# GradientSpaces/LivingScenes

Measured on AMD Instinct MI355X. Metric: object-instances/sec (encode+match+register), N=1024 pts, higher is better.
Workload: dtype f32 (GEMM products as two-piece f16 splits on the f16 matrix cores, fp32 accumulate: as accurate against fp64 as an fp32 FMA chain)

## Files before the change

livingscenes_amd/csrc/edge_fused.hip:

```cpp
#include "ls_common.h"

namespace ls {

constexpr int FK = 16;
constexpr int FND = 32;
typedef _Float16 fh8_t __attribute__((ext_vector_type(8)));
typedef _Float16 fh2_t __attribute__((ext_vector_type(2)));
typedef float ff2_t __attribute__((ext_vector_type(2)));
typedef float ff16_t __attribute__((ext_vector_type(16)));

__device__ __forceinline__ void fsplit_pair(ff2_t v, unsigned& h, unsigned& l) {
    const fh2_t hv = __builtin_convertvector(v, fh2_t);
    const fh2_t lv = __builtin_convertvector(v - __builtin_convertvector(hv, ff2_t), fh2_t);
    h = __builtin_bit_cast(unsigned, hv);
    l = __builtin_bit_cast(unsigned, lv);
}
__device__ __forceinline__ void fpow2(float amax, float& s, int& e_inv) {
    unsigned be = (__float_as_uint(amax) >> 23) & 0xffu;
    be = be < 15u ? 15u : be;
    s = __uint_as_float((268u - be) << 23);
    e_inv = (int)be - 14 - 127;
}
template <int CTRL>
__device__ __forceinline__ float fdpp_max(float v) {
    return fmaxf(v, __int_as_float(__builtin_amdgcn_update_dpp(__float_as_int(v), __float_as_int(v), CTRL, 0xF, 0xF, false)));
}
template <int CTRL>
__device__ __forceinline__ float fdpp_add(float v) {
    return v + __int_as_float(__builtin_amdgcn_update_dpp(0, __float_as_int(v), CTRL, 0xF, 0xF, true));
}
__device__ __forceinline__ float fquad_sum(float v) { return fdpp_add<0x4E>(fdpp_add<0xB1>(v)); }
__device__ __forceinline__ float fquad_max(float v) { return fdpp_max<0x4E>(fdpp_max<0xB1>(v)); }
__device__ __forceinline__ float finv_fro(float ss) { return __builtin_amdgcn_rsqf(fmaxf(ss, 1e-24f)); }

__global__ __launch_bounds__(64) void edge_ft_presplit_w_kernel(const float* __restrict__ W, int Co, int Cin, int KS, uint4* __restrict__ planes,
                                                                int* __restrict__ wexp) {
    const int T = blockIdx.x / KS, ks = blockIdx.x % KS, lane = threadIdx.x;
    const int head = T / 5, p = T % 5, r = lane & 31;
    const float* wr = W + ((size_t)(2 * p + (r >> 4)) * Co + 16 * head + (r & 15)) * Cin;
    float am = 0.f;
    for (int c = 0; c < Cin; ++c) am = fmaxf(am, fabsf(wr[c]));
    float sc;
    int e;
    fpow2(am, sc, e);
    if (ks == 0 && lane < 32) wexp[T * 32 + r] = e;
    const int k = ks * 16 + 8 * (lane >> 5);
    uint4 h, l;
    fsplit_pair(ff2_t{wr[k] * sc, wr[k + 1] * sc}, h.x, l.x);
    fsplit_pair(ff2_t{wr[k + 2] * sc, wr[k + 3] * sc}, h.y, l.y);
    fsplit_pair(ff2_t{wr[k + 4] * sc, wr[k + 5] * sc}, h.z, l.z);
    fsplit_pair(ff2_t{wr[k + 6] * sc, wr[k + 7] * sc}, h.w, l.w);
    planes[((size_t)blockIdx.x * 2) * 64 + lane] = h;
    planes[((size_t)blockIdx.x * 2 + 1) * 64 + lane] = l;
}
size_t edge_ft_w_bytes(int Co, int Cin) { return (size_t)(Co / 16) * 5 * (Cin / 16) * 2 * 64 * sizeof(uint4) + (size_t)(Co / 16) * 5 * 32 * sizeof(int); }
int edge_ft_presplit_w_launch(const float* W, int Co, int Cin, void* planes, hipStream_t st) {
    const int tiles = (Co / 16) * 5, KS = Cin / 16;
    hipLaunchKernelGGL(edge_ft_presplit_w_kernel, dim3(tiles * KS), dim3(64), 0, st, W, Co, Cin, KS, (uint4*)planes,
                       (int*)((uint4*)planes + (size_t)tiles * KS * 128));
    LS_LAUNCH_CHECK();
    return LS_OK;
}

template <int KS>
__global__ __launch_bounds__(256) void edge_ft_prep_a_kernel(const float* __restrict__ cur, const int32_t* __restrict__ rows, int Ns, int Nd,
                                                             uint4* __restrict__ planes, int* __restrict__ aexp) {
    constexpr int CIN = KS * 16, KPW = KS / 4;
    __shared__ float lmax[4][32];
    const int lane = threadIdx.x & 63, w = threadIdx.x >> 6, j = lane & 31, h = lane >> 5;
    const int R = blockIdx.x * 32 + j;
    size_t src = (size_t)R;
    if (rows) {
        const int x = R % 3, pn = R / 3, b = pn / Nd;
        src = ((size_t)b * Ns + rows[pn]) * 3 + x;
    }
    const float* rp = cur + src * CIN + (w * KPW) * 16 + h * 8;
    float4 v[KPW][2];
    float am = 0.f;
#pragma unroll
    for (int kk = 0; kk < KPW; ++kk) {
        v[kk][0] = *reinterpret_cast<const float4*>(rp + kk * 16);
        v[kk][1] = *reinterpret_cast<const float4*>(rp + kk * 16 + 4);
    }
#pragma unroll
    for (int kk = 0; kk < KPW; ++kk)
#pragma unroll
        for (int u = 0; u < 2; ++u)
            am = fmaxf(am, fmaxf(fmaxf(fabsf(v[kk][u].x), fabsf(v[kk][u].y)), fmaxf(fabsf(v[kk][u].z), fabsf(v[kk][u].w))));
    am = fmaxf(am, __shfl_xor(am, 32, 64));
    if (h == 0) lmax[w][j] = am;
    __syncthreads();
    am = fmaxf(fmaxf(lmax[0][j], lmax[1][j]), fmaxf(lmax[2][j], lmax[3][j]));
    float sc;
    int e;
    fpow2(am, sc, e);
    if (w == 0 && h == 0) aexp[R] = e;
#pragma unroll
    for (int kk = 0; kk < KPW; ++kk) {
        uint4 hh, ll;
        fsplit_pair(ff2_t{v[kk][0].x * sc, v[kk][0].y * sc}, hh.x, ll.x);
        fsplit_pair(ff2_t{v[kk][0].z * sc, v[kk][0].w * sc}, hh.y, ll.y);
        fsplit_pair(ff2_t{v[kk][1].x * sc, v[kk][1].y * sc}, hh.z, ll.z);
        fsplit_pair(ff2_t{v[kk][1].z * sc, v[kk][1].w * sc}, hh.w, ll.w);
        uint4* op = planes + (((size_t)blockIdx.x * KS + w * KPW + kk) * 2) * 64 + lane;
        op[0] = hh;
        op[64] = ll;
    }
}

struct FT43 { float4 x, y, z; };
__device__ __forceinline__ FT43 ft_lds43(const float* p, int sld) {
    FT43 r;
    r.x = *reinterpret_cast<const float4*>(p);
    r.y = *reinterpret_cast<const float4*>(p + sld);
    r.z = *reinterpret_cast<const float4*>(p + 2 * sld);
    return r;
}
__device__ __forceinline__ FT43 ft_add43(const FT43& a, const FT43& b) {
    FT43 r;
    r.x = make_float4(a.x.x + b.x.x, a.x.y + b.x.y, a.x.z + b.x.z, a.x.w + b.x.w);
    r.y = make_float4(a.y.x + b.y.x, a.y.y + b.y.y, a.y.z + b.y.z, a.y.w + b.y.w);
    r.z = make_float4(a.z.x + b.z.x, a.z.y + b.z.y, a.z.z + b.z.z, a.z.w + b.z.w);
    return r;
}
__device__ __forceinline__ void ft_act43(FT43& y, const FT43& k, float oms) {
    vn_act(y.x.x, y.y.x, y.z.x, k.x.x, k.y.x, k.z.x, oms);
    vn_act(y.x.y, y.y.y, y.z.y, k.x.y, k.y.y, k.z.y, oms);
    vn_act(y.x.z, y.y.z, y.z.z, k.x.z, k.y.z, k.z.z, oms);
    vn_act(y.x.w, y.y.w, y.z.w, k.x.w, k.y.w, k.z.w, oms);
}
__device__ __forceinline__ float ft_dot43(const FT43& a, const FT43& b) {
    float s = a.x.x * b.x.x;
    s = __builtin_fmaf(a.y.x, b.y.x, s); s = __builtin_fmaf(a.z.x, b.z.x, s);
    s = __builtin_fmaf(a.x.y, b.x.y, s); s = __builtin_fmaf(a.y.y, b.y.y, s); s = __builtin_fmaf(a.z.y, b.z.y, s);
    s = __builtin_fmaf(a.x.z, b.x.z, s); s = __builtin_fmaf(a.y.z, b.y.z, s); s = __builtin_fmaf(a.z.z, b.z.z, s);
    s = __builtin_fmaf(a.x.w, b.x.w, s); s = __builtin_fmaf(a.y.w, b.y.w, s); s = __builtin_fmaf(a.z.w, b.z.w, s);
    return s;
}
__device__ __forceinline__ void ft_fma43(FT43& acc, float w, const FT43& y) {
    acc.x.x = __builtin_fmaf(w, y.x.x, acc.x.x); acc.x.y = __builtin_fmaf(w, y.x.y, acc.x.y); acc.x.z = __builtin_fmaf(w, y.x.z, acc.x.z); acc.x.w = __builtin_fmaf(w, y.x.w, acc.x.w);
    acc.y.x = __builtin_fmaf(w, y.y.x, acc.y.x); acc.y.y = __builtin_fmaf(w, y.y.y, acc.y.y); acc.y.z = __builtin_fmaf(w, y.y.z, acc.y.z); acc.y.w = __builtin_fmaf(w, y.y.w, acc.y.w);
    acc.z.x = __builtin_fmaf(w, y.z.x, acc.z.x); acc.z.y = __builtin_fmaf(w, y.z.y, acc.z.y); acc.z.z = __builtin_fmaf(w, y.z.z, acc.z.z); acc.z.w = __builtin_fmaf(w, y.z.w, acc.z.w);
}

template <int KS>
struct FtJob { const uint4* a_planes; const int* a_exp; int mt0; int MT; int p; float* slab; int sld; };

template <int KS, int MPU>
__device__ __forceinline__ void ft_gemm_unit(const FtJob<KS>& jb, int tile0, int hl, int T, const uint4* __restrict__ wplanes, const int* __restrict__ wexp, int lane) {
    const char* ab = reinterpret_cast<const char*>(jb.a_planes + ((size_t)(jb.mt0 + tile0) * KS * 2) * 64);
    const char* wb = reinterpret_cast<const char*>(wplanes + ((size_t)T * KS * 2) * 64);
    const int we = wexp[T * 32 + (lane & 31)];
    ff16_t acc[MPU];
#pragma unroll
    for (int m = 0; m < MPU; ++m)
#pragma unroll
        for (int r = 0; r < 16; ++r) acc[m][r] = 0.f;
    unsigned voff = (unsigned)lane * 16u;
    constexpr int KB = 2;
    struct Stage { fh8_t ah[MPU][KB], al[MPU][KB], bh[KB], bl[KB]; };
    auto load_stage = [&](Stage& sg, int k0) {
        asm volatile("" : "+v"(voff));
#pragma unroll
        for (int u = 0; u < KB; ++u) {
            sg.bh[u] = __builtin_bit_cast(fh8_t, *reinterpret_cast<const uint4*>(wb + (size_t)((k0 + u) * 2) * 1024 + voff));
            sg.bl[u] = __builtin_bit_cast(fh8_t, *reinterpret_cast<const uint4*>(wb + (size_t)((k0 + u) * 2 + 1) * 1024 + voff));
#pragma unroll
            for (int m = 0; m < MPU; ++m) {
                sg.ah[m][u] = __builtin_bit_cast(fh8_t, *reinterpret_cast<const uint4*>(ab + (size_t)((m * KS + k0 + u) * 2) * 1024 + voff));
                sg.al[m][u] = __builtin_bit_cast(fh8_t, *reinterpret_cast<const uint4*>(ab + (size_t)((m * KS + k0 + u) * 2 + 1) * 1024 + voff));
            }
        }
    };
    auto run_stage = [&](const Stage& sg) {
#pragma unroll
        for (int u = 0; u < KB; ++u)
#pragma unroll
            for (int m = 0; m < MPU; ++m) {
                acc[m] = __builtin_amdgcn_mfma_f32_32x32x16_f16(sg.al[m][u], sg.bh[u], acc[m], 0, 0, 0);
                acc[m] = __builtin_amdgcn_mfma_f32_32x32x16_f16(sg.ah[m][u], sg.bh[u], acc[m], 0, 0, 0);
                acc[m] = __builtin_amdgcn_mfma_f32_32x32x16_f16(sg.ah[m][u], sg.bl[u], acc[m], 0, 0, 0);
            }
#pragma unroll
        for (int m = 0; m < MPU; ++m) asm volatile("" : "+v"(acc[m])::"memory");
    };
#pragma unroll
    for (int k0 = 0; k0 < KS; k0 += KB) {
        Stage sg;
        load_stage(sg, k0);
        __builtin_amdgcn_sched_barrier(0);
        run_stage(sg);
    }
#pragma unroll
    for (int m = 0; m < MPU; ++m) {
        const int mt = tile0 + m;
        const int row0 = 32 * mt + 4 * (lane >> 5);
        float* sp = jb.slab + (size_t)row0 * jb.sld + hl * 32 + (lane & 31);
        const int* ae = jb.a_exp + (jb.mt0 + mt) * 32 + 4 * (lane >> 5);
#pragma unroll
        for (int r = 0; r < 16; ++r) {
            const int dr = (r & 3) + 8 * (r >> 2);
            sp[dr * jb.sld] = __builtin_ldexpf(acc[m][r], ae[dr] + we);
        }
    }
}
template <int KS, int HG, int NJ>
__device__ __forceinline__ void ft_gemm_phase_g3(const FtJob<KS> (&jobs)[NJ], const uint4* __restrict__ wplanes, const int* __restrict__ wexp, int head0,
                                                 int wave, int lane) {
    if constexpr (NJ == 2 && HG == 1) {
        if (jobs[0].MT == 12 && jobs[1].MT == 3) {
            ft_gemm_unit<KS, 3>(jobs[0], 3 * wave, 0, head0 * 5 + jobs[0].p, wplanes, wexp, lane);
            if (wave < 3) ft_gemm_unit<KS, 1>(jobs[1], wave, 0, head0 * 5 + jobs[1].p, wplanes, wexp, lane);
            return;
        }
    }
    int total = 0;
#pragma unroll
    for (int j = 0; j < NJ; ++j) total += (jobs[j].MT / 3) * HG;
    for (int t = wave; t < total; t += 4) {
        int j = 0, off = t;
#pragma unroll
        for (int q = 0; q < NJ - 1; ++q)
            if (j == q && off >= (jobs[q].MT / 3) * HG) { off -= (jobs[q].MT / 3) * HG; j = q + 1; }
        FtJob<KS> jb = jobs[0];
#pragma unroll
        for (int q = 1; q < NJ; ++q)
            if (j == q) jb = jobs[q];
        const int ng = jb.MT / 3, hl = off / ng, g = off - hl * ng;
        ft_gemm_unit<KS, 3>(jb, 3 * g, hl, (head0 + hl) * 5 + jb.p, wplanes, wexp, lane);
    }
}

template <int KS, int HG, int NJ>
__device__ __forceinline__ void ft_gemm_phase_shared(const FtJob<KS> (&jobs)[NJ], const uint4* __restrict__ wplanes, const int* __restrict__ wexp, int head0,
                                                     int wave, int lane, uint4* ring) {
    const bool has_unit = wave < NJ * HG;
    const int j = has_unit ? wave / HG : 0, hl = wave % HG;
    FtJob<KS> jb = jobs[0];
#pragma unroll
    for (int q = 1; q < NJ; ++q)
        if (j == q) jb = jobs[q];
    const int T = (head0 + hl) * 5 + jb.p;
    const char* ab = reinterpret_cast<const char*>(jobs[0].a_planes + ((size_t)jobs[0].mt0 * KS * 2) * 64);
    const char* wb = reinterpret_cast<const char*>(wplanes + ((size_t)T * KS * 2) * 64);
    const int we = wexp[T * 32 + (lane & 31)];
    ff16_t acc[3];
#pragma unroll
    for (int m = 0; m < 3; ++m)
#pragma unroll
        for (int r = 0; r < 16; ++r) acc[m][r] = 0.f;
    unsigned voff = (unsigned)lane * 16u;
    auto a_addr = [&](int k0, int f) { const int u = f / 6, m = (f % 6) / 2, pl = f % 2; return ab + (size_t)((m * KS + k0 + u) * 2 + pl) * 1024 + voff; };
    constexpr int NB = KS / 2;
    uint4 sA_r0, sA_r1, sA_r2, sA_w0, sA_w1, sA_w2, sA_w3, sB_r0, sB_r1, sB_r2, sB_w0, sB_w1, sB_w2, sB_w3, sC_r0, sC_r1, sC_r2, sC_w0, sC_w1, sC_w2, sC_w3;
#define LS_FT_LOAD_BATCH(S, K0)                                                                           \
    {                                                                                                     \
        asm volatile("" : "+v"(voff));                                                                    \
        S##_r0 = *reinterpret_cast<const uint4*>(a_addr((K0), wave * 3 + 0));                             \
        S##_r1 = *reinterpret_cast<const uint4*>(a_addr((K0), wave * 3 + 1));                             \
        S##_r2 = *reinterpret_cast<const uint4*>(a_addr((K0), wave * 3 + 2));                             \
        S##_w0 = *reinterpret_cast<const uint4*>(wb + (size_t)(((K0) + 0) * 2) * 1024 + voff);            \
        S##_w1 = *reinterpret_cast<const uint4*>(wb + (size_t)(((K0) + 0) * 2 + 1) * 1024 + voff);        \
        S##_w2 = *reinterpret_cast<const uint4*>(wb + (size_t)(((K0) + 1) * 2) * 1024 + voff);            \
        S##_w3 = *reinterpret_cast<const uint4*>(wb + (size_t)(((K0) + 1) * 2 + 1) * 1024 + voff);        \
    }
#define LS_FT_STEP(S, BI)                                                                                                                          \
    {                                                                                                                                              \
        uint4* rb = ring + ((BI) & 1) * 12 * 64;                                                                                                   \
        rb[(wave * 3 + 0) * 64 + lane] = S##_r0;                                                                                                   \
        rb[(wave * 3 + 1) * 64 + lane] = S##_r1;                                                                                                   \
        rb[(wave * 3 + 2) * 64 + lane] = S##_r2;                                                                                                   \
        const fh8_t bh0 = __builtin_bit_cast(fh8_t, S##_w0), bl0 = __builtin_bit_cast(fh8_t, S##_w1), bh1 = __builtin_bit_cast(fh8_t, S##_w2),     \
                    bl1 = __builtin_bit_cast(fh8_t, S##_w3);                                                                                       \
        if ((BI) + 3 < NB) LS_FT_LOAD_BATCH(S, 2 * ((BI) + 3))                                                                                     \
        __syncthreads();                                                                                                                           \
        if (has_unit) {                                                                                                                            \
            _Pragma("unroll") for (int u = 0; u < 2; ++u) {                                                                                        \
                const fh8_t bh = u ? bh1 : bh0, bl = u ? bl1 : bl0;                                                                                \
                _Pragma("unroll") for (int m = 0; m < 3; ++m) {                                                                                    \
                    const fh8_t ah = __builtin_bit_cast(fh8_t, rb[(u * 6 + m * 2) * 64 + lane]), al = __builtin_bit_cast(fh8_t, rb[(u * 6 + m * 2 + 1) * 64 + lane]); \
                    acc[m] = __builtin_amdgcn_mfma_f32_32x32x16_f16(al, bh, acc[m], 0, 0, 0);                                                      \
                    acc[m] = __builtin_amdgcn_mfma_f32_32x32x16_f16(ah, bh, acc[m], 0, 0, 0);                                                      \
                    acc[m] = __builtin_amdgcn_mfma_f32_32x32x16_f16(ah, bl, acc[m], 0, 0, 0);                                                      \
                }                                                                                                                                  \
            }                                                                                                                                      \
        }                                                                                                                                          \
    }
    LS_FT_LOAD_BATCH(sA, 0)
    if (1 < NB) LS_FT_LOAD_BATCH(sB, 2)
    if (2 < NB) LS_FT_LOAD_BATCH(sC, 4)
#pragma unroll
    for (int bi = 0; bi < NB; bi += 3) {
        LS_FT_STEP(sA, bi)
        if (bi + 1 < NB) LS_FT_STEP(sB, bi + 1)
        if (bi + 2 < NB) LS_FT_STEP(sC, bi + 2)
    }
#undef LS_FT_STEP
#undef LS_FT_LOAD_BATCH
    if (has_unit) {
#pragma unroll
        for (int m = 0; m < 3; ++m) {
            const int row0 = 32 * m + 4 * (lane >> 5);
            float* sp = jb.slab + (size_t)row0 * jb.sld + hl * 32 + (lane & 31);
            const int* ae = jb.a_exp + (jb.mt0 + m) * 32 + 4 * (lane >> 5);
#pragma unroll
            for (int r = 0; r < 16; ++r) {
                const int dr = (r & 3) + 8 * (r >> 2);
                sp[dr * jb.sld] = __builtin_ldexpf(acc[m][r], ae[dr] + we);
            }
        }
    }
}

template <int HG>
struct FtMap {
    int n, hl, ql, k0, kn;
    __device__ __forceinline__ FtMap(int tid) {
        ql = tid & 3;
        const int idx = tid >> 2;
        n = idx >> 1;
        if constexpr (HG == 2) { hl = idx & 1; k0 = 0; kn = FK; }
        else { hl = 0; k0 = (idx & 1) * (FK / 2); kn = FK / 2; }
    }
};

template <int CIN, int NS, int HG>
__global__ __launch_bounds__(256, 2) void edge_ft_qk_kernel(const uint4* __restrict__ a_p, const int* __restrict__ ae_p, const uint4* __restrict__ a_q,
                                                         const int* __restrict__ ae_q, const uint4* __restrict__ wplanes, const int* __restrict__ wexp,
                                                         const int32_t* __restrict__ knn, int B, int H, float oms, float* __restrict__ scores,
                                                         float* __restrict__ sskp, float* __restrict__ ssqp) {
    constexpr int KS = CIN / 16, MTP = NS * 3 / 32, MTQ = FND * 3 / 32, SLD = HG * 32 + 4;
    __shared__ __attribute__((aligned(16))) float slab_q[FND * 3 * SLD];
    __shared__ __attribute__((aligned(16))) float slab_p[NS * 3 * SLD];
    __shared__ __attribute__((aligned(16))) uint4 a_ring[NS == 32 ? 2 * 12 * 64 : 1];
    const int tid = threadIdx.x, lane = tid & 63, wave = __builtin_amdgcn_readfirstlane(tid >> 6);
    const int logical = xcd_remap(blockIdx.x, gridDim.x);
    const int ngroups = H / HG;
    const int hg = logical % ngroups, b = logical / ngroups, head0 = hg * HG;
    const FtMap<HG> mp(tid);
    const int head = head0 + mp.hl;

    {
        const FtJob<KS> jq[1] = {{a_q, ae_q, b * MTQ, MTQ, 4, slab_q, SLD}};
        if constexpr (NS == 32) ft_gemm_phase_shared<KS, HG, 1>(jq, wplanes, wexp, head0, wave, lane, a_ring);
        else ft_gemm_phase_g3<KS, HG, 1>(jq, wplanes, wexp, head0, wave, lane);
    }
    __syncthreads();
    const int c4 = mp.hl * 32 + mp.ql * 4;
    FT43 qf = ft_lds43(slab_q + (size_t)(3 * mp.n) * SLD + c4, SLD);
    {
        const FT43 kd = ft_lds43(slab_q + (size_t)(3 * mp.n) * SLD + c4 + 16, SLD);
        ft_act43(qf, kd, oms);
    }
    const float ssq = fquad_sum(ft_dot43(qf, qf));
    if (mp.ql == 0 && mp.k0 == 0) ssqp[((size_t)b * H + head) * FND + mp.n] = ssq;
    int nb[FK];
    {
        const int4* kp = reinterpret_cast<const int4*>(knn + ((size_t)b * FND + mp.n) * FK + mp.k0);
#pragma unroll
        for (int u = 0; u < FK / 4; ++u)
            if (4 * u < mp.kn) { const int4 v = kp[u]; nb[4 * u] = v.x; nb[4 * u + 1] = v.y; nb[4 * u + 2] = v.z; nb[4 * u + 3] = v.w; }
    }
    __syncthreads();

    {
        const FtJob<KS> jk[2] = {{a_p, ae_p, b * MTP, MTP, 1, slab_p, SLD}, {a_q, ae_q, b * MTQ, MTQ, 3, slab_q, SLD}};
        if constexpr (NS == 32) ft_gemm_phase_shared<KS, HG, 2>(jk, wplanes, wexp, head0, wave, lane, a_ring);
        else ft_gemm_phase_g3<KS, HG, 2>(jk, wplanes, wexp, head0, wave, lane);
    }
    __syncthreads();
    {
        const FT43 ql = ft_lds43(slab_q + (size_t)(3 * mp.n) * SLD + c4, SLD), qd = ft_lds43(slab_q + (size_t)(3 * mp.n) * SLD + c4 + 16, SLD);
        float* so = scores + (((size_t)b * H + head) * FND + mp.n) * FK + mp.k0;
        float* ko = sskp + (((size_t)b * H + head) * FND + mp.n) * FK + mp.k0;
#pragma unroll
        for (int k = 0; k < FK; ++k) {
            if (k < mp.kn) {
                const float* pr = slab_p + (size_t)(3 * nb[k]) * SLD + c4;
                FT43 y = ft_add43(ft_lds43(pr, SLD), ql);
                const FT43 kd = ft_add43(ft_lds43(pr + 16, SLD), qd);
                ft_act43(y, kd, oms);
                const float s2 = fquad_sum(ft_dot43(y, y));
                const float a = fquad_sum(ft_dot43(y, qf));
                if (mp.ql == 0) { so[k] = a; ko[k] = s2; }
            }
        }
    }
}

__global__ __launch_bounds__(256) void edge_ft_norms_kernel(const float* __restrict__ sskp, const float* __restrict__ ssqp, int H, float* __restrict__ invk,
                                                            float* __restrict__ invq) {
    LS_LATENCY_CRITICAL();
    const int b = blockIdx.x, tid = threadIdx.x;
    for (int e = tid; e < FND * FK + FND; e += 256) {
        const bool isk = e < FND * FK;
        const int stride = isk ? FND * FK : FND;
        const float* sp = isk ? sskp + (size_t)b * H * FND * FK + e : ssqp + (size_t)b * H * FND + (e - FND * FK);
        float s = 0.f;
        int h = 0;
        for (; h + 8 <= H; h += 8) {
            float v[8];
#pragma unroll
            for (int u = 0; u < 8; ++u) v[u] = sp[(size_t)(h + u) * stride];
#pragma unroll
            for (int u = 0; u < 8; ++u) s += v[u];
        }
        for (; h < H; ++h) s += sp[(size_t)h * stride];
        if (isk) invk[(size_t)b * FND * FK + e] = finv_fro(s);
        else invq[(size_t)b * FND + (e - FND * FK)] = finv_fro(s);
    }
}

template <int CIN, int NS, int HG>
__global__ __launch_bounds__(256, 2) void edge_ft_v_kernel(const uint4* __restrict__ a_p, const int* __restrict__ ae_p, const uint4* __restrict__ a_q,
                                                        const int* __restrict__ ae_q, const uint4* __restrict__ wplanes, const int* __restrict__ wexp,
                                                        const int32_t* __restrict__ knn, int B, int H, float oms, float inv_sqrt_dk,
                                                        const float* __restrict__ scores, const float* __restrict__ invk, const float* __restrict__ invq,
                                                        float* __restrict__ out, int Co, float* __restrict__ rowmax, int rm_parts, float* __restrict__ colsum) {
    constexpr int KS = CIN / 16, MTP = NS * 3 / 32, MTQ = FND * 3 / 32, SLD = HG * 32 + 4;
    __shared__ __attribute__((aligned(16))) float slab_q[FND * 3 * SLD];
    __shared__ __attribute__((aligned(16))) float slab_p[NS * 3 * SLD];
    __shared__ __attribute__((aligned(16))) uint4 a_ring[NS == 32 ? 2 * 12 * 64 : 1];
    const int tid = threadIdx.x, lane = tid & 63, wave = __builtin_amdgcn_readfirstlane(tid >> 6);
    const int logical = xcd_remap(blockIdx.x, gridDim.x);
    const int ngroups = H / HG;
    const int hg = logical % ngroups, b = logical / ngroups, head0 = hg * HG;
    const FtMap<HG> mp(tid);
    const int head = head0 + mp.hl;

    int nb[FK];
    float4 sraw[FK / 4], ik4[FK / 4];
    float iq;
    {
        const int4* kp = reinterpret_cast<const int4*>(knn + ((size_t)b * FND + mp.n) * FK);
        const float4* sp = reinterpret_cast<const float4*>(scores + (((size_t)b * H + head) * FND + mp.n) * FK);
        const float4* ip = reinterpret_cast<const float4*>(invk + ((size_t)b * FND + mp.n) * FK);
#pragma unroll
        for (int u = 0; u < FK / 4; ++u) {
            const int4 v = kp[u];
            nb[4 * u] = v.x; nb[4 * u + 1] = v.y; nb[4 * u + 2] = v.z; nb[4 * u + 3] = v.w;
            sraw[u] = sp[u];
            ik4[u] = ip[u];
        }
        iq = invq[(size_t)b * FND + mp.n] * inv_sqrt_dk;
    }
    {
        const FtJob<KS> jv[2] = {{a_p, ae_p, b * MTP, MTP, 0, slab_p, SLD}, {a_q, ae_q, b * MTQ, MTQ, 2, slab_q, SLD}};
        if constexpr (NS == 32) ft_gemm_phase_shared<KS, HG, 2>(jv, wplanes, wexp, head0, wave, lane, a_ring);
        else ft_gemm_phase_g3<KS, HG, 2>(jv, wplanes, wexp, head0, wave, lane);
    }
    __syncthreads();
    float wgt[FK];
    float sum = 0.f;
    {
        float mx = -INFINITY;
#pragma unroll
        for (int u = 0; u < FK / 4; ++u) {
            const float4 v = sraw[u], ik = ik4[u];
            wgt[4 * u] = v.x * iq * ik.x;
            wgt[4 * u + 1] = v.y * iq * ik.y;
            wgt[4 * u + 2] = v.z * iq * ik.z;
            wgt[4 * u + 3] = v.w * iq * ik.w;
        }
#pragma unroll
        for (int k = 0; k < FK; ++k) mx = fmaxf(mx, wgt[k]);
#pragma unroll
        for (int k = 0; k < FK; ++k) { wgt[k] = expf(wgt[k] - mx); sum += wgt[k]; }
    }
    const int c4 = mp.hl * 32 + mp.ql * 4;
    FT43 acc;
    acc.x = acc.y = acc.z = make_float4(0.f, 0.f, 0.f, 0.f);
    {
        const FT43 ql = ft_lds43(slab_q + (size_t)(3 * mp.n) * SLD + c4, SLD), qd = ft_lds43(slab_q + (size_t)(3 * mp.n) * SLD + c4 + 16, SLD);
#pragma unroll
        for (int k = 0; k < FK; ++k) {
            if (k >= mp.k0 && k < mp.k0 + mp.kn) {
                const float* pr = slab_p + (size_t)(3 * nb[k]) * SLD + c4;
                FT43 y = ft_add43(ft_lds43(pr, SLD), ql);
                const FT43 kd = ft_add43(ft_lds43(pr + 16, SLD), qd);
                ft_act43(y, kd, oms);
                ft_fma43(acc, wgt[k], y);
            }
        }
    }
    if constexpr (HG == 1) {
        auto comb = [&](float v) { const float o = __shfl_xor(v, 4, 64); return (tid & 4) ? o + v : v + o; };
        acc.x = make_float4(comb(acc.x.x), comb(acc.x.y), comb(acc.x.z), comb(acc.x.w));
        acc.y = make_float4(comb(acc.y.x), comb(acc.y.y), comb(acc.y.z), comb(acc.y.w));
        acc.z = make_float4(comb(acc.z.x), comb(acc.z.y), comb(acc.z.z), comb(acc.z.w));
    }
    const float inv = 1.0f / sum;
    const float4 ox = make_float4(acc.x.x * inv, acc.x.y * inv, acc.x.z * inv, acc.x.w * inv);
    const float4 oy = make_float4(acc.y.x * inv, acc.y.y * inv, acc.y.z * inv, acc.y.w * inv);
    const float4 oz = make_float4(acc.z.x * inv, acc.z.y * inv, acc.z.z * inv, acc.z.w * inv);
    const bool writer = HG == 2 || (tid & 4) == 0;
    if (writer) {
        float* op = out + ((size_t)b * FND + mp.n) * 3 * Co + head * 16 + mp.ql * 4;
        *reinterpret_cast<float4*>(op) = ox;
        *reinterpret_cast<float4*>(op + Co) = oy;
        *reinterpret_cast<float4*>(op + 2 * Co) = oz;
    }
    if (rowmax) {
        auto amax4 = [](const float4& v) { return fmaxf(fmaxf(fabsf(v.x), fabsf(v.y)), fmaxf(fabsf(v.z), fabsf(v.w))); };
        float rx = fquad_max(amax4(ox)), ry = fquad_max(amax4(oy)), rz = fquad_max(amax4(oz));
        if constexpr (HG == 2) {
            rx = fmaxf(rx, __shfl_xor(rx, 4, 64)); ry = fmaxf(ry, __shfl_xor(ry, 4, 64)); rz = fmaxf(rz, __shfl_xor(rz, 4, 64));
        }
        if ((tid & 7) == 0) {
            float* rp = rowmax + (((size_t)b * FND + mp.n) * 3) * rm_parts + hg;
            rp[0] = rx; rp[rm_parts] = ry; rp[2 * rm_parts] = rz;
        }
    }
    if (colsum) {
        constexpr int CW = HG * 16;
        __syncthreads();
        if (writer) {
            float* cp = slab_q + mp.n * 3 * CW + mp.hl * 16 + mp.ql * 4;
            *reinterpret_cast<float4*>(cp) = ox;
            *reinterpret_cast<float4*>(cp + CW) = oy;
            *reinterpret_cast<float4*>(cp + 2 * CW) = oz;
        }
        __syncthreads();
        if (tid < 3 * CW) {
            float a = 0.f;
#pragma unroll 8
            for (int n = 0; n < FND; ++n) a += slab_q[n * 3 * CW + tid];
            const int ax = tid / CW, c = tid - ax * CW;
            colsum[((size_t)b * 3 + ax) * Co + head0 * 16 + c] = a;
        }
    }
}

bool edge_ft_supported(int Co, int Cin, int Ns, int Nd, int head_c, bool has_rows) {
    if (head_c != 16 || Nd != FND) return false;
    if (Cin == 128 && Ns == 128 && has_rows && Co % 16 == 0) return true;
    if (Cin == 256 && Ns == 32 && !has_rows && Co % 32 == 0) return true;
    return false;
}
int edge_ft_heads_per_group(int Cin) { return Cin == 256 ? 2 : 1; }
size_t edge_ft_scratch_bytes(int B, int Ns, int Nd, int Cin, int Co, bool has_rows) {
    const size_t rp = (size_t)B * Ns * 3, rq = (size_t)B * Nd * 3, H = Co / 16;
    size_t s = rp * Cin * 4 + rp * 4 + 512;
    if (has_rows) s += rq * Cin * 4 + rq * 4 + 512;
    s += 2 * ((size_t)B * H * Nd * FK * 4 + 256) + (size_t)B * H * Nd * 4 + 256;
    s += (size_t)B * Nd * FK * 4 + 256 + (size_t)B * Nd * 4 + 256;
    return s;
}
struct FtScratch { uint4* a_p; int* ae_p; uint4* a_q; int* ae_q; float* scores; float* sskp; float* ssqp; float* invk; float* invq; };
static FtScratch ft_layout(void* scratch, int B, int Ns, int Nd, int Cin, int Co, bool has_rows) {
    auto up = [](size_t v) { return (v + 255) & ~(size_t)255; };
    const size_t rp = (size_t)B * Ns * 3, rq = (size_t)B * Nd * 3, H = Co / 16;
    char* c = (char*)scratch;
    FtScratch s;
    size_t off = 0;
    s.a_p = (uint4*)(c + off); off = up(off + rp * Cin * 4);
    s.ae_p = (int*)(c + off); off = up(off + rp * 4);
    if (has_rows) {
        s.a_q = (uint4*)(c + off); off = up(off + rq * Cin * 4);
        s.ae_q = (int*)(c + off); off = up(off + rq * 4);
    } else { s.a_q = s.a_p; s.ae_q = s.ae_p; }
    s.scores = (float*)(c + off); off = up(off + (size_t)B * H * Nd * FK * 4);
    s.sskp = (float*)(c + off); off = up(off + (size_t)B * H * Nd * FK * 4);
    s.ssqp = (float*)(c + off); off = up(off + (size_t)B * H * Nd * 4);
    s.invk = (float*)(c + off); off = up(off + (size_t)B * Nd * FK * 4);
    s.invq = (float*)(c + off);
    return s;
}
int edge_ft_prep_launch(const float* cur, const int32_t* dst_rows, int B, int Ns, int Nd, int Cin, int Co, void* scratch, hipStream_t st) {
    const bool has_rows = dst_rows != nullptr;
    LS_REQUIRE(edge_ft_supported(Co, Cin, Ns, Nd, 16, has_rows), "edge_ft_prep: unsupported shape (Co=%d Cin=%d Ns=%d Nd=%d)", Co, Cin, Ns, Nd);
    const FtScratch s = ft_layout(scratch, B, Ns, Nd, Cin, Co, has_rows);
    if (Cin == 128) {
        hipLaunchKernelGGL(edge_ft_prep_a_kernel<8>, dim3(B * Ns * 3 / 32), dim3(256), 0, st, cur, (const int32_t*)nullptr, Ns, Nd, s.a_p, s.ae_p);
        LS_LAUNCH_CHECK();
        hipLaunchKernelGGL(edge_ft_prep_a_kernel<8>, dim3(B * Nd * 3 / 32), dim3(256), 0, st, cur, dst_rows, Ns, Nd, s.a_q, s.ae_q);
    } else {
        hipLaunchKernelGGL(edge_ft_prep_a_kernel<16>, dim3(B * Ns * 3 / 32), dim3(256), 0, st, cur, (const int32_t*)nullptr, Ns, Nd, s.a_p, s.ae_p);
    }
    LS_LAUNCH_CHECK();
    return LS_OK;
}
int edge_ft_attn_launch(const void* wplanes, const int32_t* knn, bool has_rows, int B, int Ns, int Nd, int Cin, int Co, float neg_slope, void* scratch,
                        float* out, float* rowmax, hipStream_t st, float* colsum) {
    LS_REQUIRE(edge_ft_supported(Co, Cin, Ns, Nd, 16, has_rows) && wplanes, "edge_ft_attn: unsupported shape (Co=%d Cin=%d Ns=%d Nd=%d)", Co, Cin, Ns, Nd);
    const FtScratch s = ft_layout(scratch, B, Ns, Nd, Cin, Co, has_rows);
    const int H = Co / 16, HG = edge_ft_heads_per_group(Cin), KS = Cin / 16;
    const uint4* wp = (const uint4*)wplanes;
    const int* we = (const int*)(wp + (size_t)H * 5 * KS * 128);
    const float oms = 1.0f - neg_slope, isd = 1.0f / sqrtf(3.0f * 16);
    const dim3 grid((H / HG) * B);
    if (Cin == 128) {
        hipLaunchKernelGGL((edge_ft_qk_kernel<128, 128, 1>), grid, dim3(256), 0, st, s.a_p, s.ae_p, s.a_q, s.ae_q, wp, we, knn, B, H, oms, s.scores, s.sskp, s.ssqp);
        LS_LAUNCH_CHECK();
        hipLaunchKernelGGL(edge_ft_norms_kernel, dim3(B), dim3(256), 0, st, s.sskp, s.ssqp, H, s.invk, s.invq);
        LS_LAUNCH_CHECK();
        hipLaunchKernelGGL((edge_ft_v_kernel<128, 128, 1>), grid, dim3(256), 0, st, s.a_p, s.ae_p, s.a_q, s.ae_q, wp, we, knn, B, H, oms, isd, s.scores, s.invk,
                           s.invq, out, Co, rowmax, H / HG, colsum);
    } else {
        hipLaunchKernelGGL((edge_ft_qk_kernel<256, 32, 2>), grid, dim3(256), 0, st, s.a_p, s.ae_p, s.a_q, s.ae_q, wp, we, knn, B, H, oms, s.scores, s.sskp, s.ssqp);
        LS_LAUNCH_CHECK();
        hipLaunchKernelGGL(edge_ft_norms_kernel, dim3(B), dim3(256), 0, st, s.sskp, s.ssqp, H, s.invk, s.invq);
        LS_LAUNCH_CHECK();
        hipLaunchKernelGGL((edge_ft_v_kernel<256, 32, 2>), grid, dim3(256), 0, st, s.a_p, s.ae_p, s.a_q, s.ae_q, wp, we, knn, B, H, oms, isd, s.scores, s.invk,
                           s.invq, out, Co, rowmax, H / HG, colsum);
    }
    LS_LAUNCH_CHECK();
    return LS_OK;
}
int edge_ft_rowmax_parts(int Co, int Cin) { return Co / 16 / edge_ft_heads_per_group(Cin); }

}
```

Measured before the change: 56910.

## Fuse query and key edge GEMM phases, sharing A-tile loads across weights

Merges the two separate projection GEMM phases into one pass. Each A tile is now multiplied against two weight sets in the same K loop, so activations are loaded once. The accumulator for the projection that would overwrite slab_q is kept in registers and written only after the first slab_q consumers have read it. This removes a second pass over the A planes, along with its barriers and pipeline ramp. The cost is more live accumulators (up to five 32x32 tiles per wave), which raises register pressure under launch_bounds(256,2), plus some work imbalance between odd and even waves.

```diff
diff --git a/livingscenes_amd/csrc/edge_fused.hip b/livingscenes_amd/csrc/edge_fused.hip
--- a/livingscenes_amd/csrc/edge_fused.hip
+++ b/livingscenes_amd/csrc/edge_fused.hip
@@ -146,25 +146,41 @@
 template <int KS>
 struct FtJob { const uint4* a_planes; const int* a_exp; int mt0; int MT; int p; float* slab; int sld; };
 
-template <int KS, int MPU>
-__device__ __forceinline__ void ft_gemm_unit(const FtJob<KS>& jb, int tile0, int hl, int T, const uint4* __restrict__ wplanes, const int* __restrict__ wexp, int lane) {
+__device__ __forceinline__ void ft_store_tile(float* slab, int sld, const int* a_exp, int mt_abs, int mt, int hl, int we, const ff16_t& acc, int lane) {
+    const int row0 = 32 * mt + 4 * (lane >> 5);
+    float* sp = slab + (size_t)row0 * sld + hl * 32 + (lane & 31);
+    const int* ae = a_exp + mt_abs * 32 + 4 * (lane >> 5);
+#pragma unroll
+    for (int r = 0; r < 16; ++r) {
+        const int dr = (r & 3) + 8 * (r >> 2);
+        sp[dr * sld] = __builtin_ldexpf(acc[r], ae[dr] + we);
+    }
+}
+template <int KS, int MPU, int NW>
+__device__ __forceinline__ void ft_gemm_acc(const FtJob<KS>& jb, int tile0, const int (&T)[NW], const uint4* __restrict__ wplanes, int lane,
+                                            ff16_t (&acc)[NW][MPU]) {
     const char* ab = reinterpret_cast<const char*>(jb.a_planes + ((size_t)(jb.mt0 + tile0) * KS * 2) * 64);
-    const char* wb = reinterpret_cast<const char*>(wplanes + ((size_t)T * KS * 2) * 64);
-    const int we = wexp[T * 32 + (lane & 31)];
-    ff16_t acc[MPU];
-#pragma unroll
-    for (int m = 0; m < MPU; ++m)
-#pragma unroll
-        for (int r = 0; r < 16; ++r) acc[m][r] = 0.f;
+    const char* wb[NW];
+#pragma unroll
+    for (int w = 0; w < NW; ++w) wb[w] = reinterpret_cast<const char*>(wplanes + ((size_t)T[w] * KS * 2) * 64);
+#pragma unroll
+    for (int w = 0; w < NW; ++w)
+#pragma unroll
+        for (int m = 0; m < MPU; ++m)
+#pragma unroll
+            for (int r = 0; r < 16; ++r) acc[w][m][r] = 0.f;
     unsigned voff = (unsigned)lane * 16u;
     constexpr int KB = 2;
-    struct Stage { fh8_t ah[MPU][KB], al[MPU][KB], bh[KB], bl[KB]; };
+    struct Stage { fh8_t ah[MPU][KB], al[MPU][KB], bh[NW][KB], bl[NW][KB]; };
     auto load_stage = [&](Stage& sg, int k0) {
         asm volatile("" : "+v"(voff));
 #pragma unroll
         for (int u = 0; u < KB; ++u) {
-            sg.bh[u] = __builtin_bit_cast(fh8_t, *reinterpret_cast<const uint4*>(wb + (size_t)((k0 + u) * 2) * 1024 + voff));
-            sg.bl[u] = __builtin_bit_cast(fh8_t, *reinterpret_cast<const uint4*>(wb + (size_t)((k0 + u) * 2 + 1) * 1024 + voff));
+#pragma unroll
+            for (int w = 0; w < NW; ++w) {
+                sg.bh[w][u] = __builtin_bit_cast(fh8_t, *reinterpret_cast<const uint4*>(wb[w] + (size_t)((k0 + u) * 2) * 1024 + voff));
+                sg.bl[w][u] = __builtin_bit_cast(fh8_t, *reinterpret_cast<const uint4*>(wb[w] + (size_t)((k0 + u) * 2 + 1) * 1024 + voff));
+            }
 #pragma unroll
             for (int m = 0; m < MPU; ++m) {
                 sg.ah[m][u] = __builtin_bit_cast(fh8_t, *reinterpret_cast<const uint4*>(ab + (size_t)((m * KS + k0 + u) * 2) * 1024 + voff));
@@ -176,13 +192,17 @@
 #pragma unroll
         for (int u = 0; u < KB; ++u)
 #pragma unroll
-            for (int m = 0; m < MPU; ++m) {
-                acc[m] = __builtin_amdgcn_mfma_f32_32x32x16_f16(sg.al[m][u], sg.bh[u], acc[m], 0, 0, 0);
-                acc[m] = __builtin_amdgcn_mfma_f32_32x32x16_f16(sg.ah[m][u], sg.bh[u], acc[m], 0, 0, 0);
-                acc[m] = __builtin_amdgcn_mfma_f32_32x32x16_f16(sg.ah[m][u], sg.bl[u], acc[m], 0, 0, 0);
-            }
-#pragma unroll
-        for (int m = 0; m < MPU; ++m) asm volatile("" : "+v"(acc[m])::"memory");
+            for (int w = 0; w < NW; ++w)
+#pragma unroll
+                for (int m = 0; m < MPU; ++m) {
+                    acc[w][m] = __builtin_amdgcn_mfma_f32_32x32x16_f16(sg.al[m][u], sg.bh[w][u], acc[w][m], 0, 0, 0);
+                    acc[w][m] = __builtin_amdgcn_mfma_f32_32x32x16_f16(sg.ah[m][u], sg.bh[w][u], acc[w][m], 0, 0, 0);
+                    acc[w][m] = __builtin_amdgcn_mfma_f32_32x32x16_f16(sg.ah[m][u], sg.bl[w][u], acc[w][m], 0, 0, 0);
+                }
+#pragma unroll
+        for (int w = 0; w < NW; ++w)
+#pragma unroll
+            for (int m = 0; m < MPU; ++m) asm volatile("" : "+v"(acc[w][m])::"memory");
     };
 #pragma unroll
     for (int k0 = 0; k0 < KS; k0 += KB) {
@@ -191,18 +211,15 @@
         __builtin_amdgcn_sched_barrier(0);
         run_stage(sg);
     }
-#pragma unroll
-    for (int m = 0; m < MPU; ++m) {
-        const int mt = tile0 + m;
-        const int row0 = 32 * mt + 4 * (lane >> 5);
-        float* sp = jb.slab + (size_t)row0 * jb.sld + hl * 32 + (lane & 31);
-        const int* ae = jb.a_exp + (jb.mt0 + mt) * 32 + 4 * (lane >> 5);
-#pragma unroll
-        for (int r = 0; r < 16; ++r) {
-            const int dr = (r & 3) + 8 * (r >> 2);
-            sp[dr * jb.sld] = __builtin_ldexpf(acc[m][r], ae[dr] + we);
-        }
-    }
+}
+template <int KS, int MPU>
+__device__ __forceinline__ void ft_gemm_unit(const FtJob<KS>& jb, int tile0, int hl, int T, const uint4* __restrict__ wplanes, const int* __restrict__ wexp, int lane) {
+    const int we = wexp[T * 32 + (lane & 31)];
+    const int Ts[1] = {T};
+    ff16_t acc[1][MPU];
+    ft_gemm_acc<KS, MPU, 1>(jb, tile0, Ts, wplanes, lane, acc);
+#pragma unroll
+    for (int m = 0; m < MPU; ++m) ft_store_tile(jb.slab, jb.sld, jb.a_exp, jb.mt0 + tile0 + m, tile0 + m, hl, we, acc[0][m], lane);
 }
 template <int KS, int HG, int NJ>
 __device__ __forceinline__ void ft_gemm_phase_g3(const FtJob<KS> (&jobs)[NJ], const uint4* __restrict__ wplanes, const int* __restrict__ wexp, int head0,
@@ -312,6 +329,99 @@
     }
 }
 
+__device__ __forceinline__ int ft_qk_first(int wave) { return 3 * (wave >> 1) + 2 * (wave & 1); }
+__device__ __forceinline__ int ft_qk_second(int wave) { return 3 * (wave >> 1) + 1; }
+__device__ __forceinline__ int ft_qk_p(int u) { return (u >> 1) == 0 ? 4 : (u >> 1) == 1 ? 1 : 3; }
+template <int KS>
+__device__ __forceinline__ void ft_gemm_qk_shared(const uint4* __restrict__ a_planes, int mt0, const uint4* __restrict__ wplanes, int head0, int wave, int lane,
+                                                  uint4* ring, ff16_t (&acc)[5]) {
+    const int uF = ft_qk_first(wave), uS = ft_qk_second(wave);
+    const bool odd = (wave & 1) != 0;
+    const int TF = (head0 + (uF & 1)) * 5 + ft_qk_p(uF), TS = (head0 + (uS & 1)) * 5 + ft_qk_p(uS);
+    const char* ab = reinterpret_cast<const char*>(a_planes + ((size_t)mt0 * KS * 2) * 64);
+    const char* wf = reinterpret_cast<const char*>(wplanes + ((size_t)TF * KS * 2) * 64);
+    const char* ws = reinterpret_cast<const char*>(wplanes + ((size_t)TS * KS * 2) * 64);
+#pragma unroll
+    for (int s = 0; s < 5; ++s)
+#pragma unroll
+        for (int r = 0; r < 16; ++r) acc[s][r] = 0.f;
+    unsigned voff = (unsigned)lane * 16u;
+    auto a_addr = [&](int k0, int f) { const int u = f / 6, m = (f % 6) / 2, pl = f % 2; return ab + (size_t)((m * KS + k0 + u) * 2 + pl) * 1024 + voff; };
+    constexpr int NB = KS / 2;
+    uint4 sA_r0, sA_r1, sA_r2, sA_f0, sA_f1, sA_f2, sA_f3, sA_s0, sA_s1, sA_s2, sA_s3;
+    uint4 sB_r0, sB_r1, sB_r2, sB_f0, sB_f1, sB_f2, sB_f3, sB_s0, sB_s1, sB_s2, sB_s3;
+#define LS_FT_LOAD_BATCH(S, K0)                                                                           \
+    {                                                                                                     \
+        asm volatile("" : "+v"(voff));                                                                    \
+        S##_r0 = *reinterpret_cast<const uint4*>(a_addr((K0), wave * 3 + 0));                             \
+        S##_r1 = *reinterpret_cast<const uint4*>(a_addr((K0), wave * 3 + 1));                             \
+        S##_r2 = *reinterpret_cast<const uint4*>(a_addr((K0), wave * 3 + 2));                             \
+        S##_f0 = *reinterpret_cast<const uint4*>(wf + (size_t)(((K0) + 0) * 2) * 1024 + voff);            \
+        S##_f1 = *reinterpret_cast<const uint4*>(wf + (size_t)(((K0) + 0) * 2 + 1) * 1024 + voff);        \
+        S##_f2 = *reinterpret_cast<const uint4*>(wf + (size_t)(((K0) + 1) * 2) * 1024 + voff);            \
+        S##_f3 = *reinterpret_cast<const uint4*>(wf + (size_t)(((K0) + 1) * 2 + 1) * 1024 + voff);        \
+        S##_s0 = *reinterpret_cast<const uint4*>(ws + (size_t)(((K0) + 0) * 2) * 1024 + voff);            \
+        S##_s1 = *reinterpret_cast<const uint4*>(ws + (size_t)(((K0) + 0) * 2 + 1) * 1024 + voff);        \
+        S##_s2 = *reinterpret_cast<const uint4*>(ws + (size_t)(((K0) + 1) * 2) * 1024 + voff);            \
+        S##_s3 = *reinterpret_cast<const uint4*>(ws + (size_t)(((K0) + 1) * 2 + 1) * 1024 + voff);        \
+    }
+#define LS_FT_MFMA3(ACC, AL, AH, BH, BL)                                                                  \
+    {                                                                                                     \
+        ACC = __builtin_amdgcn_mfma_f32_32x32x16_f16(AL, BH, ACC, 0, 0, 0);                               \
+        ACC = __builtin_amdgcn_mfma_f32_32x32x16_f16(AH, BH, ACC, 0, 0, 0);                               \
+        ACC = __builtin_amdgcn_mfma_f32_32x32x16_f16(AH, BL, ACC, 0, 0, 0);                               \
+    }
+#define LS_FT_STEP(S, BI)                                                                                                                          \
+    {                                                                                                                                              \
+        uint4* rb = ring + ((BI) & 1) * 12 * 64;                                                                                                   \
+        rb[(wave * 3 + 0) * 64 + lane] = S##_r0;                                                                                                   \
+        rb[(wave * 3 + 1) * 64 + lane] = S##_r1;                                                                                                   \
+        rb[(wave * 3 + 2) * 64 + lane] = S##_r2;                                                                                                   \
+        const fh8_t fh0 = __builtin_bit_cast(fh8_t, S##_f0), fl0 = __builtin_bit_cast(fh8_t, S##_f1), fh1 = __builtin_bit_cast(fh8_t, S##_f2),     \
+                    fl1 = __builtin_bit_cast(fh8_t, S##_f3);                                                                                       \
+        const fh8_t sh0 = __builtin_bit_cast(fh8_t, S##_s0), sl0 = __builtin_bit_cast(fh8_t, S##_s1), sh1 = __builtin_bit_cast(fh8_t, S##_s2),     \
+                    sl1 = __builtin_bit_cast(fh8_t, S##_s3);                                                                                       \
+        if ((BI) + 2 < NB) LS_FT_LOAD_BATCH(S, 2 * ((BI) + 2))                                                                                     \
+        __syncthreads();                                                                                                                           \
+        _Pragma("unroll") for (int u = 0; u < 2; ++u) {                                                                                            \
+            const fh8_t fh = u ? fh1 : fh0, fl = u ? fl1 : fl0, sh = u ? sh1 : sh0, sl = u ? sl1 : sl0;                                            \
+            fh8_t ah[3], al[3];                                                                                                                    \
+            _Pragma("unroll") for (int m = 0; m < 3; ++m) {                                                                                        \
+                ah[m] = __builtin_bit_cast(fh8_t, rb[(u * 6 + m * 2) * 64 + lane]);                                                                \
+                al[m] = __builtin_bit_cast(fh8_t, rb[(u * 6 + m * 2 + 1) * 64 + lane]);                                                            \
+            }                                                                                                                                      \
+            _Pragma("unroll") for (int m = 0; m < 3; ++m) LS_FT_MFMA3(acc[m], al[m], ah[m], fh, fl)                                                 \
+            LS_FT_MFMA3(acc[3], (odd ? al[2] : al[0]), (odd ? ah[2] : ah[0]), sh, sl)                                                              \
+            if (!odd) LS_FT_MFMA3(acc[4], al[1], ah[1], sh, sl)                                                                                    \
+        }                                                                                                                                          \
+        _Pragma("unroll") for (int s = 0; s < 5; ++s) asm volatile("" : "+v"(acc[s])::"memory");                                                 \
+    }
+    LS_FT_LOAD_BATCH(sA, 0)
+    if (1 < NB) LS_FT_LOAD_BATCH(sB, 2)
+#pragma unroll
+    for (int bi = 0; bi < NB; bi += 2) {
+        LS_FT_STEP(sA, bi)
+        if (bi + 1 < NB) LS_FT_STEP(sB, bi + 1)
+    }
+#undef LS_FT_STEP
+#undef LS_FT_MFMA3
+#undef LS_FT_LOAD_BATCH
+}
+template <int SLD>
+__device__ __forceinline__ void ft_qk_store_slots(const ff16_t (&acc)[5], bool deferred, const int* __restrict__ a_exp, int mt0, const int* __restrict__ wexp,
+                                                  int head0, int wave, int lane, float* slab_q, float* slab_p) {
+    const int uF = ft_qk_first(wave), uS = ft_qk_second(wave);
+    const bool odd = (wave & 1) != 0;
+#pragma unroll
+    for (int s = 0; s < 5; ++s) {
+        if (s == 4 && odd) continue;
+        const int u = s < 3 ? uF : uS, m = s < 3 ? s : s == 3 ? (odd ? 2 : 0) : 1;
+        if (((u >> 1) == 2) != deferred) continue;
+        const int T = (head0 + (u & 1)) * 5 + ft_qk_p(u);
+        ft_store_tile((u >> 1) == 1 ? slab_p : slab_q, SLD, a_exp, mt0 + m, m, u & 1, wexp[T * 32 + (lane & 31)], acc[s], lane);
+    }
+}
+
 template <int HG>
 struct FtMap {
     int n, hl, ql, k0, kn;
@@ -340,10 +450,20 @@
     const FtMap<HG> mp(tid);
     const int head = head0 + mp.hl;
 
-    {
-        const FtJob<KS> jq[1] = {{a_q, ae_q, b * MTQ, MTQ, 4, slab_q, SLD}};
-        if constexpr (NS == 32) ft_gemm_phase_shared<KS, HG, 1>(jq, wplanes, wexp, head0, wave, lane, a_ring);
-        else ft_gemm_phase_g3<KS, HG, 1>(jq, wplanes, wexp, head0, wave, lane);
+    ff16_t acc6[NS == 32 ? 5 : 1];
+    ff16_t acc5[2][1];
+    if constexpr (NS == 32) {
+        ft_gemm_qk_shared<KS>(a_q, b * MTQ, wplanes, head0, wave, lane, a_ring, acc6);
+        ft_qk_store_slots<SLD>(acc6, false, ae_q, b * MTQ, wexp, head0, wave, lane, slab_q, slab_p);
+    } else {
+        const FtJob<KS> jp = {a_p, ae_p, b * MTP, MTP, 1, slab_p, SLD}, jq = {a_q, ae_q, b * MTQ, MTQ, 4, slab_q, SLD};
+        static_assert(HG == 1 && MTP == 12 && MTQ == 3, "layer 5's plan: one head, four source groups, three destination M-tiles");
+        ft_gemm_unit<KS, 3>(jp, 3 * wave, 0, head0 * 5 + 1, wplanes, wexp, lane);
+        if (wave < 3) {
+            const int Ts[2] = {head0 * 5 + 4, head0 * 5 + 3};
+            ft_gemm_acc<KS, 1, 2>(jq, wave, Ts, wplanes, lane, acc5);
+            ft_store_tile(slab_q, SLD, ae_q, b * MTQ + wave, wave, 0, wexp[Ts[0] * 32 + (lane & 31)], acc5[0][0], lane);
+        }
     }
     __syncthreads();
     const int c4 = mp.hl * 32 + mp.ql * 4;
@@ -362,12 +482,8 @@
             if (4 * u < mp.kn) { const int4 v = kp[u]; nb[4 * u] = v.x; nb[4 * u + 1] = v.y; nb[4 * u + 2] = v.z; nb[4 * u + 3] = v.w; }
     }
     __syncthreads();
-
-    {
-        const FtJob<KS> jk[2] = {{a_p, ae_p, b * MTP, MTP, 1, slab_p, SLD}, {a_q, ae_q, b * MTQ, MTQ, 3, slab_q, SLD}};
-        if constexpr (NS == 32) ft_gemm_phase_shared<KS, HG, 2>(jk, wplanes, wexp, head0, wave, lane, a_ring);
-        else ft_gemm_phase_g3<KS, HG, 2>(jk, wplanes, wexp, head0, wave, lane);
-    }
+    if constexpr (NS == 32) ft_qk_store_slots<SLD>(acc6, true, ae_q, b * MTQ, wexp, head0, wave, lane, slab_q, slab_p);
+    else if (wave < 3) ft_store_tile(slab_q, SLD, ae_q, b * MTQ + wave, wave, 0, wexp[(head0 * 5 + 3) * 32 + (lane & 31)], acc5[1][0], lane);
     __syncthreads();
     {
         const FT43 ql = ft_lds43(slab_q + (size_t)(3 * mp.n) * SLD + c4, SLD), qd = ft_lds43(slab_q + (size_t)(3 * mp.n) * SLD + c4 + 16, SLD);
```

Result: no change. 57280 (median of 6 runs) (+0.6%).
